# mclarsen/cuZFP

Measured on AMD Instinct MI355X. Metric: GB/s input encoded+decoded (device-resident), 3D f32 fixed-rate; % HBM peak, higher is better.
Workload: dtype f32; 1 GPU; 3d_float32_256^3_rate8; maxbits=512, parallelism=z-slab x1, stream_bytes_per_gpu=16777216

## Files before the change

### cuzfp_amd/csrc/zfp_block.hpp

```cpp
#pragma once

#include <math.h>
#include <stdint.h>

#if defined(__HIPCC__)
#include <hip/hip_runtime.h>
#define ZFP_HD __host__ __device__ __forceinline__
#else
#define ZFP_HD inline
#endif

#ifndef ZFP_STAMP
#define ZFP_STAMP(i)
#endif
#ifndef ZFP_COUNT_PLANE
#define ZFP_COUNT_PLANE(g0, fast, complete)
#endif
#ifndef ZFP_COUNT_PATH
#define ZFP_COUNT_PATH(id)
#endif

namespace cuzfp {


template <typename T> struct traits;
template <> struct traits<float> {
  typedef int32_t Int; typedef uint32_t UInt;
  static constexpr bool is_int = false;
  static constexpr int prec = 32, ebits = 8, ebias = 127;
};
template <> struct traits<double> {
  typedef int64_t Int; typedef uint64_t UInt;
  static constexpr bool is_int = false;
  static constexpr int prec = 64, ebits = 11, ebias = 1023;
};
template <> struct traits<int32_t> {
  typedef int32_t Int; typedef uint32_t UInt;
  static constexpr bool is_int = true;
  static constexpr int prec = 32, ebits = 0, ebias = 0;
};
template <> struct traits<int64_t> {
  typedef int64_t Int; typedef uint64_t UInt;
  static constexpr bool is_int = true;
  static constexpr int prec = 64, ebits = 0, ebias = 0;
};

template <typename UInt> struct nbmask;
template <> struct nbmask<uint32_t> { static constexpr uint32_t value = 0xaaaaaaaau; };
template <> struct nbmask<uint64_t> { static constexpr uint64_t value = 0xaaaaaaaaaaaaaaaaull; };

ZFP_HD uint64_t lowmask(unsigned n) { return n >= 64 ? ~0ull : ((1ull << n) - 1); }

struct WRaw {
  uint32_t a0, a1, a2;
};

ZFP_HD void sched_fence() {
#if defined(__HIP_DEVICE_COMPILE__)
  __builtin_amdgcn_sched_barrier(0);
#endif
}

ZFP_HD uint32_t launder(uint32_t x) {
#if defined(__HIP_DEVICE_COMPILE__)
  asm("" : "+v"(x));
#endif
  return x;
}
ZFP_HD uint32_t uniform_const(uint32_t x) {
#if defined(__HIP_DEVICE_COMPILE__)
  asm("" : "+s"(x));
#endif
  return x;
}
ZFP_HD uint64_t uniform_const64(uint64_t x) {
#if defined(__HIP_DEVICE_COMPILE__)
  asm("" : "+s"(x));
#endif
  return x;
}
ZFP_HD uint64_t launder(uint64_t x) {
#if defined(__HIP_DEVICE_COMPILE__)
  asm("" : "+v"(x));
#endif
  return x;
}

ZFP_HD unsigned ctz64(uint64_t x) { return (unsigned)__builtin_ctzll(x); }

ZFP_HD unsigned umin(unsigned a, unsigned b) { return a < b ? a : b; }


template <int DIMS> struct perm;
template <> struct perm<1> {
  ZFP_HD static constexpr int at(int i) { return i; }
};
template <> struct perm<2> {
  ZFP_HD static constexpr int at(int i) {
    return i == 0 ? 0 : i == 1 ? 1 : i == 2 ? 4 : i == 3 ? 5 : i == 4 ? 2 : i == 5 ? 8 :
           i == 6 ? 6 : i == 7 ? 9 : i == 8 ? 3 : i == 9 ? 12 : i == 10 ? 10 : i == 11 ? 7 :
           i == 12 ? 13 : i == 13 ? 11 : i == 14 ? 14 : 15;
  }
};
#define ZFP_I3(i, j, k) ((i) + 4 * ((j) + 4 * (k)))
template <> struct perm<3> {
  ZFP_HD static constexpr int at(int i) {
    constexpr int t[64] = {
      ZFP_I3(0,0,0),
      ZFP_I3(1,0,0), ZFP_I3(0,1,0), ZFP_I3(0,0,1),
      ZFP_I3(0,1,1), ZFP_I3(1,0,1), ZFP_I3(1,1,0),
      ZFP_I3(2,0,0), ZFP_I3(0,2,0), ZFP_I3(0,0,2),
      ZFP_I3(1,1,1),
      ZFP_I3(2,1,0), ZFP_I3(2,0,1), ZFP_I3(0,2,1), ZFP_I3(1,2,0), ZFP_I3(1,0,2), ZFP_I3(0,1,2),
      ZFP_I3(3,0,0), ZFP_I3(0,3,0), ZFP_I3(0,0,3),
      ZFP_I3(2,1,1), ZFP_I3(1,2,1), ZFP_I3(1,1,2),
      ZFP_I3(0,2,2), ZFP_I3(2,0,2), ZFP_I3(2,2,0),
      ZFP_I3(3,1,0), ZFP_I3(3,0,1), ZFP_I3(0,3,1), ZFP_I3(1,3,0), ZFP_I3(1,0,3), ZFP_I3(0,1,3),
      ZFP_I3(1,2,2), ZFP_I3(2,1,2), ZFP_I3(2,2,1),
      ZFP_I3(3,1,1), ZFP_I3(1,3,1), ZFP_I3(1,1,3),
      ZFP_I3(3,2,0), ZFP_I3(3,0,2), ZFP_I3(0,3,2), ZFP_I3(2,3,0), ZFP_I3(2,0,3), ZFP_I3(0,2,3),
      ZFP_I3(2,2,2),
      ZFP_I3(3,2,1), ZFP_I3(3,1,2), ZFP_I3(1,3,2), ZFP_I3(2,3,1), ZFP_I3(2,1,3), ZFP_I3(1,2,3),
      ZFP_I3(0,3,3), ZFP_I3(3,0,3), ZFP_I3(3,3,0),
      ZFP_I3(3,2,2), ZFP_I3(2,3,2), ZFP_I3(2,2,3),
      ZFP_I3(1,3,3), ZFP_I3(3,1,3), ZFP_I3(3,3,1),
      ZFP_I3(2,3,3), ZFP_I3(3,2,3), ZFP_I3(3,3,2),
      ZFP_I3(3,3,3)};
    return t[i];
  }
};
#undef ZFP_I3

template <int... I> struct seq {};
template <int N, int... I> struct seq_gen : seq_gen<N - 1, N - 1, I...> {};
template <int... I> struct seq_gen<0, I...> { typedef seq<I...> type; };
template <int N> using make_seq = typename seq_gen<N>::type;
template <int DIMS, int I> struct pidx { static constexpr int value = perm<DIMS>::at(I); };

template <int DIMS, typename UInt, int... I>
ZFP_HD void permute_fwd_add(const UInt* q, UInt* u, UInt nb, seq<I...>) {
  ((u[I] = q[pidx<DIMS, I>::value] + nb), ...);
}
ZFP_HD uint32_t from_negabinary(uint32_t u, uint32_t nb) {
#if defined(__HIP_DEVICE_COMPILE__)
  uint32_t r;
  asm("v_xad_u32 %0, %1, %2, %3" : "=v"(r) : "v"(u), "s"(nb), "v"(0u - nb));
  return r;
#else
  return (u ^ nb) - nb;
#endif
}
ZFP_HD uint64_t from_negabinary(uint64_t u, uint64_t nb) { return (u ^ nb) - nb; }

template <int DIMS, typename UInt, int... I>
ZFP_HD void permute_inv(const UInt* u, UInt* q, UInt nb, seq<I...>) {
  ((q[pidx<DIMS, I>::value] = from_negabinary(u[I], nb)), ...);
}
template <int DIMS, typename UInt, int... I>
ZFP_HD void permute_inv_copy(const UInt* u, UInt* q, seq<I...>) {
  ((q[pidx<DIMS, I>::value] = u[I]), ...);
}
template <int DIMS, typename UInt, int... I>
ZFP_HD void permute_inv_sub(const UInt* u, UInt* q, UInt nb, seq<I...>) {
  ((q[pidx<DIMS, I>::value] = u[I] - nb), ...);
}

template <int DIMS>
ZFP_HD unsigned precision(int emax, int prec) {
  int p = emax + 1074 + 2 * (DIMS + 1);
  p = p < 0 ? 0 : p;
  return (unsigned)(p < prec ? p : prec);
}


ZFP_HD uint32_t asr1(uint32_t v) { return (uint32_t)((int32_t)v >> 1); }
ZFP_HD uint64_t asr1(uint64_t v) { return (uint64_t)((int64_t)v >> 1); }

template <typename UInt>
ZFP_HD void fwd_lift(UInt& x, UInt& y, UInt& z, UInt& w) {
  x += w; x = asr1(x); w -= x;
  z += y; z = asr1(z); y -= z;
  x += z; x = asr1(x); z -= x;
  w += y; w = asr1(w); y -= w;
  w += asr1(y); y -= asr1(w);
}

template <typename UInt>
ZFP_HD void inv_lift(UInt& x, UInt& y, UInt& z, UInt& w) {
  UInt t;
  y += asr1(w); w -= asr1(y);
  t = w - y; y += w; w = t;
  t = x - z; z += x; x = t;
  t = z - y; y += z; z = t;
  t = x - w; w += x; x = t;
}

template <int DIMS, typename UInt>
ZFP_HD void fwd_xform(UInt* p) {
  if constexpr (DIMS == 1) {
    fwd_lift(p[0], p[1], p[2], p[3]);
  } else if constexpr (DIMS == 2) {
#pragma unroll
    for (int y = 0; y < 4; y++) fwd_lift(p[4 * y], p[4 * y + 1], p[4 * y + 2], p[4 * y + 3]);
#pragma unroll
    for (int x = 0; x < 4; x++) fwd_lift(p[x], p[x + 4], p[x + 8], p[x + 12]);
  } else {
#pragma unroll
    for (int zy = 0; zy < 16; zy++) fwd_lift(p[4 * zy], p[4 * zy + 1], p[4 * zy + 2], p[4 * zy + 3]);
#pragma unroll
    for (int z = 0; z < 4; z++)
#pragma unroll
      for (int x = 0; x < 4; x++) {
        UInt* q = p + 16 * z + x;
        fwd_lift(q[0], q[4], q[8], q[12]);
      }
#pragma unroll
    for (int yx = 0; yx < 16; yx++) fwd_lift(p[yx], p[yx + 16], p[yx + 32], p[yx + 48]);
  }
}

template <int DIMS, typename UInt>
ZFP_HD void inv_xform(UInt* p) {
  if constexpr (DIMS == 1) {
    inv_lift(p[0], p[1], p[2], p[3]);
  } else if constexpr (DIMS == 2) {
#pragma unroll
    for (int x = 0; x < 4; x++) inv_lift(p[x], p[x + 4], p[x + 8], p[x + 12]);
#pragma unroll
    for (int y = 0; y < 4; y++) inv_lift(p[4 * y], p[4 * y + 1], p[4 * y + 2], p[4 * y + 3]);
  } else {
#pragma unroll
    for (int yx = 0; yx < 16; yx++) inv_lift(p[yx], p[yx + 16], p[yx + 32], p[yx + 48]);
#pragma unroll
    for (int z = 0; z < 4; z++)
#pragma unroll
      for (int x = 0; x < 4; x++) {
        UInt* q = p + 16 * z + x;
        inv_lift(q[0], q[4], q[8], q[12]);
      }
#pragma unroll
    for (int zy = 0; zy < 16; zy++) inv_lift(p[4 * zy], p[4 * zy + 1], p[4 * zy + 2], p[4 * zy + 3]);
  }
}


ZFP_HD uint32_t bfi_v(uint32_t m, uint32_t a, uint32_t b) {
#if defined(__HIP_DEVICE_COMPILE__)
  uint32_t r;
  asm("v_bfi_b32 %0, %1, %2, %3" : "=v"(r) : "v"(m), "v"(a), "v"(b));
  return r;
#else
  return (a & m) | (b & ~m);
#endif
}

ZFP_HD uint32_t bfi(uint32_t m, uint32_t a, uint32_t b) {
#if defined(__HIP_DEVICE_COMPILE__)
  uint32_t r;
  asm("v_bfi_b32 %0, %1, %2, %3" : "=v"(r) : "s"(m), "v"(a), "v"(b));
  return r;
#else
  return (a & m) | (b & ~m);
#endif
}

ZFP_HD uint32_t nbfi(uint32_t m, uint32_t a, uint32_t b) {
#if defined(__HIP_DEVICE_COMPILE__)
  uint32_t r;
  asm("v_bitop3_b32 %0, %1, %2, %3 bitop3:0x35" : "=v"(r) : "s"(m), "v"(a), "v"(b));
  return r;
#else
  return ~((a & m) | (b & ~m));
#endif
}

ZFP_HD uint32_t bfi_notb(uint32_t m, uint32_t a, uint32_t b) {
#if defined(__HIP_DEVICE_COMPILE__)
  uint32_t r;
  asm("v_bitop3_b32 %0, %1, %2, %3 bitop3:0xc5" : "=v"(r) : "s"(m), "v"(a), "v"(b));
  return r;
#else
  return (a & m) | (~b & ~m);
#endif
}

ZFP_HD uint32_t perm_bytes(uint32_t b, uint32_t a, uint32_t sel) {
#if defined(__HIP_DEVICE_COMPILE__)
  return __builtin_amdgcn_perm(b, a, sel);
#else
  const uint64_t v = (uint64_t)a | ((uint64_t)b << 32);
  uint32_t r = 0;
  for (int i = 0; i < 4; i++) r |= (uint32_t)((v >> (8 * ((sel >> (8 * i)) & 7))) & 0xff) << (8 * i);
  return r;
#endif
}

enum { kInvNone = 0, kOddWords = 1, kOddBits = 2 };

template <int J>
ZFP_HD uint32_t opaque_shift() {
#if defined(__HIP_DEVICE_COMPILE__)
  uint32_t s;
  asm("s_mov_b32 %0, %1" : "=s"(s) : "i"(J));
  return s;
#else
  return J;
#endif
}
template <int J>
ZFP_HD void shl2(uint32_t& x, uint32_t& y, uint32_t sj) {
  const uint64_t r = ((uint64_t)x | ((uint64_t)y << 32)) << sj;
  x = (uint32_t)r;
  y = (uint32_t)(r >> 32);
}
template <int J>
ZFP_HD void shr2(uint32_t& x, uint32_t& y, uint32_t sj) {
  const uint64_t r = ((uint64_t)x | ((uint64_t)y << 32)) >> sj;
  x = (uint32_t)r;
  y = (uint32_t)(r >> 32);
}

template <int J, int INV = kInvNone>
ZFP_HD void transpose_stage(uint32_t* a, int rows, int r0 = 0) {
  constexpr uint32_t m = J == 16 ? 0x0000ffffu : J == 8 ? 0x00ff00ffu : J == 4 ? 0x0f0f0f0fu
                       : J == 2 ? 0x33333333u : 0x55555555u;
  if constexpr (J <= 4) {
    constexpr int D = J == 1 ? 2 : 1;
    const uint32_t sj = opaque_shift<J>();
#pragma unroll
    for (int i = 0; i < 32; i++) {
      if (i < r0 || i >= rows || (i & J) || (i & D)) continue;
      const int i2 = i + D;
      uint32_t h1 = a[i + J], h2 = a[i2 + J], l1 = a[i], l2 = a[i2];
      const uint32_t H1 = h1, H2 = h2;
      shl2<J>(h1, h2, sj);
      shr2<J>(l1, l2, sj);
      if constexpr (INV == kOddBits) {
        a[i] = bfi_notb(m, a[i], h1);
        a[i2] = bfi_notb(m, a[i2], h2);
        a[i + J] = bfi_notb(m, l1, H1);
        a[i2 + J] = bfi_notb(m, l2, H2);
      } else {
        a[i] = bfi(m, a[i], h1);
        a[i2] = bfi(m, a[i2], h2);
        a[i + J] = INV == kOddWords ? nbfi(m, l1, H1) : bfi(m, l1, H1);
        a[i2 + J] = INV == kOddWords ? nbfi(m, l2, H2) : bfi(m, l2, H2);
      }
    }
    return;
  }
#pragma unroll
  for (int i = 0; i < 32; i++) {
    if (i < r0 || i >= rows || (i & J)) continue;
    const uint32_t lo = a[i], hi = a[i + J];
    if constexpr (J == 16) {
      a[i] = perm_bytes(hi, lo, 0x05040100u);
      a[i + J] = perm_bytes(hi, lo, 0x07060302u);
    } else if constexpr (J == 8) {
      a[i] = perm_bytes(hi, lo, 0x06020400u);
      a[i + J] = perm_bytes(hi, lo, 0x07030501u);
    } else {
      if constexpr (INV == kOddBits) {
        a[i] = bfi_notb(m, lo, hi << J);
        a[i + J] = bfi_notb(m, lo >> J, hi);
      } else {
        a[i] = bfi(m, lo, hi << J);
        a[i + J] = INV == kOddWords ? nbfi(m, lo >> J, hi) : bfi(m, lo >> J, hi);
      }
    }
  }
}

template <int R, int INV = kInvNone>
ZFP_HD void transpose_tiles(uint32_t* a) {
  if constexpr (R >= 32) transpose_stage<16>(a, R);
  if constexpr (R >= 16) transpose_stage<8>(a, R);
  if constexpr (R >= 8) transpose_stage<4>(a, R);
  if constexpr (R >= 4) transpose_stage<2>(a, R);
  if constexpr (R >= 2) transpose_stage<1, INV>(a, R);
}

template <int H, int G, int R, bool VEC> struct plane_words;
template <int H, int G, int R> struct plane_words<H, G, R, false> {
  uint32_t a[H][G][R];
  ZFP_HD uint32_t get(int h, int g, int r) const { return a[h][g][r]; }
  ZFP_HD void set(int h, int g, int r, uint32_t x) { a[h][g][r] = x; }
  ZFP_HD void zero() {
#pragma unroll
    for (int h = 0; h < H; h++)
#pragma unroll
      for (int g = 0; g < G; g++)
#pragma unroll
        for (int r = 0; r < R; r++) a[h][g][r] = 0u;
  }
};
template <int H, int G, int R> struct plane_words<H, G, R, true> {
  typedef uint32_t vec __attribute__((ext_vector_type(R)));
  vec v[H][G];
  ZFP_HD uint32_t get(int h, int g, int r) const { return v[h][g][r]; }
  ZFP_HD void set(int h, int g, int r, uint32_t x) { v[h][g][r] = x; }
  ZFP_HD void zero() {
#pragma unroll
    for (int h = 0; h < H; h++)
#pragma unroll
      for (int g = 0; g < G; g++) v[h][g] = (vec)0u;
  }
};

template <typename UInt, int DIMS> struct planes {
  static constexpr int N = 1 << (2 * DIMS);
  static constexpr int H = sizeof(UInt) / 4;
  static constexpr int R = N < 32 ? N : 32;
  static constexpr int G = N / R;
  plane_words<H, G, R, (H == 2)> w;

  template <bool NEG_ODD = false>
  ZFP_HD void load(const UInt* u) {
    uint32_t t[H][N];
#pragma unroll
    for (int i = 0; i < N; i++) {
      t[0][i] = (uint32_t)u[i];
      if (H == 2) t[H - 1][i] = (uint32_t)((uint64_t)u[i] >> 32);
    }
#pragma unroll
    for (int h = 0; h < H; h++)
#pragma unroll
      for (int g = 0; g < G; g++) transpose_tiles<R, NEG_ODD ? kOddWords : kInvNone>(&t[h][g * R]);
#pragma unroll
    for (int h = 0; h < H; h++)
#pragma unroll
      for (int g = 0; g < G; g++)
#pragma unroll
        for (int r = 0; r < R; r++) w.set(h, g, r, t[h][g * R + r]);
  }

  template <bool NEG_ODD = false>
  ZFP_HD void store(UInt* u) const {
    uint32_t t[H][N];
#pragma unroll
    for (int h = 0; h < H; h++)
#pragma unroll
      for (int g = 0; g < G; g++)
#pragma unroll
        for (int r = 0; r < R; r++) t[h][g * R + r] = w.get(h, g, r);
#pragma unroll
    for (int h = 0; h < H; h++)
#pragma unroll
      for (int g = 0; g < G; g++) transpose_tiles<R, NEG_ODD ? kOddBits : kInvNone>(&t[h][g * R]);
#pragma unroll
    for (int i = 0; i < N; i++) {
      uint64_t x = t[0][i];
      if (H == 2) x |= (uint64_t)t[H - 1][i] << 32;
      u[i] = (UInt)x;
    }
  }

  ZFP_HD void zero() { w.zero(); }

  template <bool NEG_ODD = false>
  ZFP_HD void load_split(const UInt* u) {
    static_assert(H == 2 && N == 64, "3D 64-bit blocks");
    uint32_t t[H][N];
#pragma unroll
    for (int i = 0; i < N; i++) {
      t[0][i] = (uint32_t)u[i];
      t[1][i] = (uint32_t)((uint64_t)u[i] >> 32);
    }
#pragma unroll
    for (int g = 0; g < G; g++) {
      transpose_tiles<R, NEG_ODD ? kOddWords : kInvNone>(&t[1][g * R]);
      transpose_stage<16>(&t[0][g * R], R);
    }
#pragma unroll
    for (int h = 0; h < H; h++)
#pragma unroll
      for (int g = 0; g < G; g++)
#pragma unroll
        for (int r = 0; r < R; r++) w.set(h, g, r, t[h][g * R + r]);
  }
  template <bool NEG_ODD = false, bool UPPER = true>
  ZFP_HD void lo_part() {
    constexpr int INV = NEG_ODD ? kOddWords : kInvNone;
    constexpr int r0 = UPPER ? 16 : 0, r1 = UPPER ? 32 : 16;
#pragma unroll
    for (int g = 0; g < G; g++) {
      uint32_t t[R];
#pragma unroll
      for (int r = r0; r < r1; r++) t[r] = w.get(0, g, r);
      transpose_stage<8>(t, r1, r0);
      transpose_stage<4>(t, r1, r0);
      transpose_stage<2>(t, r1, r0);
      transpose_stage<1, INV>(t, r1, r0);
#pragma unroll
      for (int r = r0; r < r1; r++) w.set(0, g, r, t[r]);
    }
  }

  template <bool NEG_ODD = false>
  ZFP_HD void load_hi(const UInt* u) {
    static_assert(DIMS == 2 && H == 1, "2D 32-bit blocks");
    uint32_t d[8];
#pragma unroll
    for (int k = 0; k < 8; k++) d[k] = perm_bytes(u[k + 8], u[k], 0x07030602u);
    transpose_tiles<8, NEG_ODD ? kOddWords : kInvNone>(d);
#pragma unroll
    for (int k = 0; k < 8; k++) {
      w.set(0, 0, k, d[k] << 16);
      w.set(0, 0, k + 8, d[k]);
    }
  }
  template <bool NEG_ODD = false>
  ZFP_HD void store_hi(UInt* q) const {
    static_assert(DIMS == 2 && H == 1, "2D 32-bit blocks");
    uint32_t d[8];
#pragma unroll
    for (int k = 0; k < 8; k++) d[k] = perm_bytes(w.get(0, 0, k + 8), w.get(0, 0, k), 0x07030602u);
    transpose_tiles<8, NEG_ODD ? kOddBits : kInvNone>(d);
#pragma unroll
    for (int k = 0; k < 8; k++) {
      if constexpr (NEG_ODD) {
        q[k] = (d[k] - 0xaaaau) << 16;
        q[k + 8] = (d[k] & 0xffff0000u) - 0xaaaa0000u;
      } else {
        q[k] = d[k] << 16;
        q[k + 8] = d[k] & 0xffff0000u;
      }
    }
  }

  template <int h> ZFP_HD uint64_t get(int c) const {
    if constexpr (N == 64) return (uint64_t)w.get(h, 0, c) | ((uint64_t)w.get(h, 1, c) << 32);
    else return (w.get(h, 0, c % R) >> (R * (c / R))) & (uint32_t)lowmask(R);
  }
  ZFP_HD uint64_t get(int k) const {
    return (k >> 5) ? get<H - 1>(k & 31) : get<0>(k & 31);
  }
  template <int h> ZFP_HD uint32_t word(int c) const { return w.get(h, 0, c % R); }

  template <int h> ZFP_HD void set(int c, uint64_t x) {
    if constexpr (N == 64) {
      w.set(h, 0, c, (uint32_t)x);
      w.set(h, 1, c, (uint32_t)(x >> 32));
    } else {
      w.set(h, 0, c % R, w.get(h, 0, c % R) | ((uint32_t)x << (R * (c / R))));
    }
  }
  ZFP_HD void set(int k, uint64_t x) {
    if (k >> 5) set<H - 1>(k & 31, x);
    else set<0>(k & 31, x);
  }
};


template <int DIMS> struct plane_word { typedef uint32_t type; };
template <> struct plane_word<3> { typedef uint64_t type; };

ZFP_HD unsigned ctz(uint32_t x) { return (unsigned)__builtin_ctz(x); }
ZFP_HD unsigned ctz(uint64_t x) { return (unsigned)__builtin_ctzll(x); }

ZFP_HD unsigned ctz64_or_64(uint64_t x) {
#if defined(__HIP_DEVICE_COMPILE__)
  unsigned lo, hi;
  asm("v_ffbl_b32 %0, %1" : "=v"(lo) : "v"((uint32_t)x));
  asm("v_ffbl_b32 %0, %1" : "=v"(hi) : "v"((uint32_t)(x >> 32)));
  hi |= 32u;
  return lo < hi ? lo : hi;
#else
  const uint32_t lo = (uint32_t)x, hi = (uint32_t)(x >> 32);
  const unsigned zl = lo ? (unsigned)__builtin_ctz(lo) : 64u;
  const unsigned zh = hi ? 32u + (unsigned)__builtin_ctz(hi) : 64u;
  return zl < zh ? zl : zh;
#endif
}

ZFP_HD int uniform(int c) {
#if defined(__HIP_DEVICE_COMPILE__)
  return __builtin_amdgcn_readfirstlane(c);
#else
  return c;
#endif
}

ZFP_HD bool any_lane(bool p) {
#if defined(__HIP_DEVICE_COMPILE__) && !defined(CUZFP_LANE_EXIT)
  return __builtin_amdgcn_ballot_w64(p) != 0;
#else
  return p;
#endif
}

#ifndef CUZFP_PRIO_T2
#define CUZFP_PRIO_T2 17
#define CUZFP_PRIO_T1 9
#define CUZFP_PRIO_T0 1
#endif
#ifndef CUZFP_DPRIO_T2
#define CUZFP_DPRIO_T2 21
#define CUZFP_DPRIO_T1 11
#define CUZFP_DPRIO_T0 (-1)
#define CUZFP_DPRIO_AFTER 2
#endif
template <typename T, typename = void> struct prio_of {
  static constexpr bool value = true;
};
template <typename T> struct prio_of<T, decltype((void)T::kPrio)> {
  static constexpr bool value = T::kPrio;
};

template <typename T, typename = void> struct zero_inline_of {
  static constexpr bool value = false;
};
template <typename T> struct zero_inline_of<T, decltype((void)T::kZeroInline)> {
  static constexpr bool value = T::kZeroInline;
};

template <typename T, typename = void> struct put32_of {
  static constexpr bool value = false;
};
template <typename T> struct put32_of<T, decltype((void)T::kPut32)> {
  static constexpr bool value = T::kPut32;
};
template <typename W>
ZFP_HD auto wr_head(W& wr, uint64_t v, unsigned n) -> decltype(wr.head(v, n)) {
  wr.head(v, n);
}
template <typename W, typename... Ignored>
ZFP_HD void wr_head(W& wr, uint64_t v, unsigned n, Ignored...) {
  wr.put(v, n);
}

template <int T2, int T1, int T0>
ZFP_HD void progress_priority(int c) {
#if defined(__HIP_DEVICE_COMPILE__) && !defined(CUZFP_NO_PRIO)
  constexpr uint32_t kAt = (1u << T2) | (1u << T1) | (T0 >= 0 ? 1u << (T0 & 31) : 0u);
  if (__builtin_expect((kAt >> (c & 31)) & 1u, 0)) {
    if (c == T2) __builtin_amdgcn_s_setprio(2);
    else if (c == T1) __builtin_amdgcn_s_setprio(1);
    else __builtin_amdgcn_s_setprio(0);
  }
#else
  (void)c;
#endif
}

constexpr uint32_t spread_entry(uint32_t b) {
  uint32_t e = 0, p = 0;
  for (int i = 0; i < 8; i++) {
    if ((b >> i) & 1u) {
      e |= 3u << p;
      p += 2;
    } else {
      p += 1;
    }
  }
  return e;
}
struct SpreadLut {
  uint32_t e[256];
};
constexpr SpreadLut make_spread_lut() {
  SpreadLut t{};
  for (uint32_t b = 0; b < 256; b++) t.e[b] = spread_entry(b);
  return t;
}

struct SpreadTab {
  uint32_t e[512];
};
constexpr SpreadTab make_spread_tab() {
  SpreadTab t{};
  for (uint32_t b = 0; b < 256; b++) {
    uint32_t pop = 0;
    for (int i = 0; i < 8; i++) pop += (b >> i) & 1u;
    t.e[b] = (((spread_entry(b) << 1) | 1u) << 5) | (pop + 8u);
    t.e[256 + b] = spread_entry(b) << 1;
  }
  return t;
}

// ... 559 lines not shown
  const uint32_t d = parsed - b1;
  const bool done = ended | ((d == 0u) & (st != 0u));
  const bool cut = !done & ((int32_t)d >= 0);
  const uint32_t P = npos - (cut ? d : 0u);
  slow = (cut & (P > q)) | (!cut & (!done | ((int32_t)d > 1) | (npos > q)));
  uint64_t ones64 = ones | ((uint64_t)(cut ? 1u : 0u) << (P & 63u));
  uint32_t np = P + (cut ? 1u : 0u), take = umin(parsed, b1);
  if (__builtin_expect(any_lane(npos > q), 0)) {
    if (npos > q) {
      uint64_t o64 = ones;
      uint32_t o = implied_end(e1, e2, q, o64);
      if (ent_pos(e1) + ent_pos(e2) <= q) o = io;
      if (o <= b1) {
        slow = false;
        ones64 = o64;
        np = q + 1u;
        take = o;
      } else if (!cut) {
        slow = true;
      }
    }
  }
  ZFP_COUNT_PATH(slow ? (npos > q ? (cut ? 11 : 12) : (cut ? 13 : (!ended ? 14 : 15))) : 10);
  const PW hi = (PW)(~0ull << m);
  const PW x = (hi & ((PW)ones64 << nf)) | (~hi & (PW)w);
  n = nf + np;
  const unsigned adv = m + take;
  rd.pos += adv;
  bits -= adv;
  return x;
}

template <int DIMS, typename PW, typename Reader>
ZFP_HD PW decode_plane_lut(unsigned& bits, unsigned& n, Reader& rd, bool& slow) {
  constexpr unsigned N = 1u << (2 * DIMS);
  const unsigned nf = n < N - 1 ? n : N - 1;
  const unsigned m = umin(nf, bits);
  uint64_t w;
  uint32_t g;
  rd.windows(m, w, g);
  uint32_t e1, e2;
  if constexpr (DIMS == 1) {
    e1 = rd.chunk1_fast(g);
    e2 = 0;
  } else {
    uint32_t sel, e2a, e2b;
    rd.chunks_fast(g, e1, sel, e2a, e2b);
    e2 = perm_sel(e2b, e2a, sel);
  }
  return lut_finish<DIMS, PW>(bits, n, rd, slow, nf, m, w, e1, e2);
}

template <int DIMS, typename PW, typename Reader>
ZFP_HD PW decode_plane_any(unsigned& n, Reader& rd) {
  constexpr unsigned N = 1u << (2 * DIMS);
  const auto pos0 = rd.pos;
  const unsigned n0 = n;
  unsigned bits = rd.end - pos0;
  bool slow;
  PW x = decode_plane_lut<DIMS, PW>(bits, n, rd, slow);
  ZFP_COUNT_PATH(slow ? 6 : 5);
  if (__builtin_expect(any_lane(slow), 0)) {
    if (slow) {
      rd.init(pos0);
      n = n0;
      bits = rd.end - pos0;
      x = decode_plane<DIMS, PW>(bits, n, rd);
    }
  }
  n = umin(n, N - 1);
  return x;
}



template <int DIMS, typename PW, typename Reader>
ZFP_HD PW decode_plane_fast_any(unsigned& n, Reader& rd) {
  constexpr unsigned N = 1u << (2 * DIMS);
  const unsigned nf = n;
  WRaw wr;
  const uint32_t g = rd.window_g(nf, wr);
  uint32_t e1, e2, sel = 0, e2a = 0, e2b = 0;
  if constexpr (DIMS == 1)
    e1 = rd.chunk1_fast(g);
  else
    rd.chunks_fast(g, e1, sel, e2a, e2b);
  sched_fence();
  rd.lds_wait();
  sched_fence();
  const uint64_t w = rd.window_w_make(wr);
  if constexpr (DIMS == 1) {
    e2 = 0;
  } else {
    e2 = perm_sel(e2b, e2a, sel);
  }
  const uint32_t S = e1 + e2;
  const uint32_t nfp = nf + ent_pos(S);
  const int32_t rare = (int32_t)(S | ((N == 64 ? nfp : launder(nfp + (64u - N))) << 25));
  if (__builtin_expect(any_lane(rare < 0), 0)) {
    const auto pos0 = rd.pos;
    ZFP_COUNT_PATH((S & kMarkerBit) ? 16 : (nfp >= N) ? 17 : 18);
    unsigned bits = rd.end - rd.pos;
    bool slow;
    PW x = lut_finish<DIMS, PW>(bits, n, rd, slow, nf, umin(nf, bits), w, e1, e2);
    n = umin(n, N - 1);
    ZFP_COUNT_PATH(slow ? 2 : 1);
    if (any_lane(slow)) {
      if (slow) {
        rd.init(pos0);
        n = nf;
        bits = rd.end - pos0;
        x = decode_plane<DIMS, PW>(bits, n, rd);
        n = umin(n, N - 1);
      }
    }
    rd.lds_wait();
    return x;
  }
  ZFP_COUNT_PATH(0);
  const uint32_t ones = ent_ones(e1) | (ent_ones(e2) << ((e1 >> kPosShift) & 31u));
  PW x;
  if constexpr (sizeof(PW) == 8) {
    x = (PW)(w ^ (((w >> nf) ^ (uint64_t)ones) << nf));
  } else {
    x = merge_at<PW>(nf, ones, w);
  }
  n = nfp;
  rd.pos = umin(rd.pos + nf + ent_used(S), rd.end);
  return x;
}

template <int H, typename UInt, int DIMS, typename Reader>
ZFP_HD int decode_half(planes<UInt, DIMS>& P, unsigned& n, Reader& rd) {
  typedef typename plane_word<DIMS>::type PW;
  int c = 31;
  for (; c >= 1; c -= 2) {
    if (!any_lane(rd.pos < rd.end)) return c;
    if constexpr (prio_of<Reader>::value)
      progress_priority<CUZFP_DPRIO_T2, CUZFP_DPRIO_T1, CUZFP_DPRIO_T0>(uniform(c));
    PW xa, xb;
    xa = decode_plane_fast_any<DIMS, PW>(n, rd);
    xb = decode_plane_fast_any<DIMS, PW>(n, rd);
    ZFP_STAMP(4);
    const int u = uniform(c);
    P.template set<H>(u, xa);
    P.template set<H>(u - 1, xb);
  }
  return c;
}

#ifndef CUZFP_F64_SPLIT
#define CUZFP_F64_SPLIT 1
#endif
#ifndef CUZFP_EAGER_ZERO
constexpr bool kLazyZero = true;
#else
constexpr bool kLazyZero = false;
#endif
template <int H, int C, typename UInt, int DIMS>
ZFP_HD void zero_fixed(planes<UInt, DIMS>& P) {
  if constexpr (C >= 0) {
    P.template set<H>(C, 0);
    zero_fixed<H, C - 1>(P);
  }
}

template <int H, int C, bool PRI = true, typename UInt, int DIMS, typename Reader>
ZFP_HD int decode_half_fixed(planes<UInt, DIMS>& P, unsigned& n, Reader& rd) {
  typedef typename plane_word<DIMS>::type PW;
  if constexpr (C >= 1) {
    if (!any_lane(rd.pos < rd.end)) {
      if constexpr (kLazyZero && DIMS == 3) zero_fixed<H, C>(P);
      return C;
    }
#if defined(__HIP_DEVICE_COMPILE__) && !defined(CUZFP_NO_PRIO)
    if constexpr (prio_of<Reader>::value && PRI) {
      if constexpr (C == CUZFP_DPRIO_T2) __builtin_amdgcn_s_setprio(2);
      else if constexpr (C == CUZFP_DPRIO_T1) __builtin_amdgcn_s_setprio(1);
      else if constexpr (C == CUZFP_DPRIO_T0) __builtin_amdgcn_s_setprio(0);
    }
#endif
    const PW xa = decode_plane_fast_any<DIMS, PW>(n, rd);
    const PW xb = decode_plane_fast_any<DIMS, PW>(n, rd);
    ZFP_STAMP(4);
    P.template set<H>(C, xa);
    P.template set<H>(C - 1, xb);
    return decode_half_fixed<H, C - 2, PRI>(P, n, rd);
  }
  return C;
}


template <int H, typename UInt, int DIMS>
ZFP_HD void zero_planes(planes<UInt, DIMS>& P, int c) {
  if constexpr (kLazyZero && DIMS == 3)
    for (; c >= 0; c--) P.template set<H>(uniform(c), 0);
}

template <typename T, typename = void> struct has_dec1d {
  static constexpr bool value = false;
};
template <typename T> struct has_dec1d<T, decltype((void)&T::dec1d)> {
  static constexpr bool value = true;
};

template <int H, int C, typename UInt, typename Reader>
ZFP_HD void decode_planes_1d(planes<UInt, 1>& P, uint32_t& n12, Reader& rd) {
  if constexpr (C >= 0) {
    if constexpr (C & 1)
      if (!any_lane(rd.pos < rd.end)) return;
    const uint32_t c = umin(rd.end - rd.pos, 7u);
    const uint32_t e = rd.dec1d((rd.bits8() << 1) | ((c << 9) | n12));
    P.template set<H>(C, e & 15u);
    rd.pos += (e >> 4) & 15u;
    n12 = e & 0x3000u;
    decode_planes_1d<H, C - 1>(P, n12, rd);
  }
}

template <typename UInt, int DIMS, typename Reader>
ZFP_HD int decode_planes(planes<UInt, DIMS>& P, unsigned budget, Reader& rd) {
  constexpr int PREC = (int)sizeof(UInt) * 8;
  unsigned n = 0;
  rd.end = rd.pos + budget;
  if constexpr (!(kLazyZero && DIMS == 3)) P.zero();
  if constexpr (PREC == 32) {
    if constexpr (DIMS == 1 && has_dec1d<Reader>::value) {
      uint32_t n12 = 0;
      decode_planes_1d<0, 31>(P, n12, rd);
      return 31;
    }
    return decode_half_fixed<0, 31>(P, n, rd);
  } else {
    if constexpr (DIMS == 1 && has_dec1d<Reader>::value) {
      uint32_t n12 = 0;
      decode_planes_1d<1, 31>(P, n12, rd);
      decode_planes_1d<0, 31>(P, n12, rd);
      return 31;
    }
    zero_planes<1>(P, decode_half<1>(P, n, rd));
    zero_planes<0>(P, decode_half<0>(P, n, rd));
  }
  return 31;
}

template <typename UInt, int N>
ZFP_HD void cut_planes(UInt* v, unsigned maxprec) {
  constexpr unsigned PREC = (unsigned)sizeof(UInt) * 8;
  if (__builtin_expect(any_lane(maxprec != PREC), 0)) {
    const UInt m = (UInt)lowmask(PREC - maxprec);
    constexpr UInt NB = nbmask<UInt>::value;
#pragma unroll
    for (int i = 0; i < N; i++) v[i] = (v[i] & ~m) | (NB & m);
  }
}


template <typename Scalar> struct fp;

template <> struct fp<float> {
  template <int N>
  ZFP_HD static int emax(const float* f) {
    float m = 0.0f;
#pragma unroll
    for (int i = 0; i < N; i++) m = fmaxf(m, fabsf(f[i]));
    uint32_t b = __float_as_uint_(m);
    int E = (int)(b >> 23);
    if (b == 0) return -127;
    return E == 255 ? 0 : E - 126;
  }
  ZFP_HD static float pow2(int e) {
    if (e > 127) return __uint_as_float_(0x7f800000u);
    if (e >= -126) return __uint_as_float_((uint32_t)(e + 127) << 23);
    if (e >= -149) return __uint_as_float_(1u << (e + 149));
    return 0.0f;
  }
  ZFP_HD static int32_t to_int(float y) {
    return fabsf(y) < 2147483648.0f ? (int32_t)y : (int32_t)0x80000000u;
  }
  ZFP_HD static float from_int(int32_t q) { return (float)q; }
  ZFP_HD static uint32_t __float_as_uint_(float f) { union { float f; uint32_t u; } c; c.f = f; return c.u; }
  ZFP_HD static float __uint_as_float_(uint32_t u) { union { float f; uint32_t u; } c; c.u = u; return c.f; }
};

template <> struct fp<double> {
  template <int N>
  ZFP_HD static int emax(const double* f) {
    double m = 0.0;
#pragma unroll
    for (int i = 0; i < N; i++) m = fmax(m, fabs(f[i]));
    uint64_t b = as_u64(m);
    int E = (int)(b >> 52);
    if (b == 0) return -1023;
    return E == 2047 ? 0 : E - 1022;
  }
  ZFP_HD static double pow2(int e) {
    if (e > 1023) return as_f64(0x7ff0000000000000ull);
    if (e >= -1022) return as_f64((uint64_t)(e + 1023) << 52);
    if (e >= -1074) return as_f64(1ull << (e + 1074));
    return 0.0;
  }
  ZFP_HD static int64_t to_int(double y) {
    return fabs(y) < 9223372036854775808.0 ? (int64_t)y : (int64_t)0x8000000000000000ull;
  }
  ZFP_HD static double from_int(int64_t q) { return (double)q; }
  ZFP_HD static uint64_t as_u64(double f) { union { double f; uint64_t u; } c; c.f = f; return c.u; }
  ZFP_HD static double as_f64(uint64_t u) { union { double f; uint64_t u; } c; c.u = u; return c.f; }
};


#if defined(__HIP_DEVICE_COMPILE__)
template <int N>
__device__ __forceinline__ float absmax_nan(const float* f) {
  constexpr int C = N >= 16 ? 4 : 1;
  float m[C];
#pragma unroll
  for (int c = 0; c < C; c++) m[c] = 0.0f;
#pragma unroll
  for (int i = 0; i < N; i += 2) {
    float& a = m[(i / 2) % C];
    asm("v_maximum3_f32 %0, |%1|, |%2|, %0" : "+v"(a) : "v"(f[i]), "v"(f[i + 1]));
  }
  if constexpr (C == 4) {
    asm("v_maximum3_f32 %0, %0, %1, %2" : "+v"(m[0]) : "v"(m[1]), "v"(m[2]));
    asm("v_maximum3_f32 %0, %0, %1, %1" : "+v"(m[0]) : "v"(m[3]));
  }
  return m[0];
}
#endif

#if defined(__HIP_DEVICE_COMPILE__)
template <int N>
__device__ __forceinline__ void quantize_f32(const float* f, float s, bool fast, uint32_t* q) {
  typedef float f2 __attribute__((ext_vector_type(2)));
  if constexpr (N <= 16) fast = !any_lane(!fast);
  if (fast) {
    const f2 ss = {s, s};
#pragma unroll
    for (int i = 0; i < N; i += 2) {
      const f2 y = f2{f[i], f[i + 1]} * ss;
      q[i] = (uint32_t)(int32_t)y.x;
      q[i + 1] = (uint32_t)(int32_t)y.y;
    }
  }
  if (fast) {
  } else {
    const float lim = 2147483648.0f;
    const uint32_t imin = 0x80000000u;
#pragma unroll
    for (int i = 0; i < N; i += 2) {
      float a = f[i], b = f[i + 1];
      uint64_t m;
      uint32_t t;
      asm("v_mul_f32 %0, %0, %4\n\t"
          "v_mul_f32 %1, %1, %4\n\t"
          "v_cmp_gt_f32_e64 vcc, %5, |%0|\n\t"
          "v_cmp_gt_f32_e64 %2, %5, |%1|\n\t"
          "v_cvt_i32_f32 %3, %0\n\t"
          "v_cndmask_b32 %0, %6, %3, vcc\n\t"
          "v_cvt_i32_f32 %3, %1\n\t"
          "v_cndmask_b32_e64 %1, %6, %3, %2"
          : "+v"(a), "+v"(b), "=&s"(m), "=&v"(t)
          : "v"(s), "v"(lim), "v"(imin)
          : "vcc");
      q[i] = __builtin_bit_cast(uint32_t, a);
      q[i + 1] = __builtin_bit_cast(uint32_t, b);
    }
  }
}
#endif

template <typename Scalar, int DIMS, typename Writer>
ZFP_HD void encode_block(const Scalar* f, unsigned maxbits, Writer& wr) {
  typedef traits<Scalar> T;
  typedef typename T::Int Int;
  typedef typename T::UInt UInt;
  constexpr int N = 1 << (2 * DIMS);
  UInt q[N];
  unsigned maxprec = T::prec;
  (void)maxbits;
  if constexpr (!T::is_int) {
#if defined(__HIP_DEVICE_COMPILE__)
    bool finite = false;
    int emax;
    if constexpr (sizeof(Scalar) == 4 && N % 2 == 0) {
      const float mx = absmax_nan<N>((const float*)f);
      finite = __builtin_isfinite(mx);
      if (__builtin_expect(finite, 1)) {
        const uint32_t bm = __builtin_bit_cast(uint32_t, mx);
        emax = bm ? (int)(bm >> 23) - 126 : -127;
      } else {
        emax = fp<Scalar>::template emax<N>((const Scalar*)f);
      }
    } else {
      emax = fp<Scalar>::template emax<N>((const Scalar*)f);
    }
#else
    const int emax = fp<Scalar>::template emax<N>((const Scalar*)f);
#endif
    ZFP_STAMP(1);
    maxprec = precision<DIMS>(emax, T::prec);
    const unsigned e = maxprec ? (unsigned)(emax + T::ebias) : 0u;
    bool zero = !e;
    if (zero) maxprec = T::prec;
    if constexpr (zero_inline_of<Writer>::value) {
      if (!any_lane(!zero)) {
        wr.finish();
        return;
      }
      wr.mark_full(zero);
    } else if (zero) {
      wr.finish();
      return;
    }
    wr_head(wr, 2ull * e + 1, T::ebits + 1);
    Scalar s = (Scalar)fp<Scalar>::pow2(T::prec - 2 - emax);
    if constexpr (zero_inline_of<Writer>::value) s = zero ? (Scalar)0 : s;
#if defined(__HIP_DEVICE_COMPILE__)
    if constexpr (sizeof(Scalar) == 4 && N % 2 == 0) {
      quantize_f32<N>((const float*)f, (float)s, finite && (emax >= -97 || zero), (uint32_t*)q);
    } else
#endif
    {
#pragma unroll
      for (int i = 0; i < N; i++) q[i] = (UInt)fp<Scalar>::to_int(s * (Scalar)f[i]);
    }
  } else {
#pragma unroll
    for (int i = 0; i < N; i++) q[i] = (UInt)(Int)f[i];
  }
  fwd_xform<DIMS>(q);
  UInt u[N];
  constexpr UInt NB = nbmask<UInt>::value;
  permute_fwd_add<DIMS>(q, u, NB, make_seq<N>());
  if constexpr (sizeof(UInt) == 8 && !T::is_int) cut_planes<UInt, N>(u, maxprec);
  ZFP_STAMP(2);
#if defined(CUZFP_PROBE) && (CUZFP_PROBE == 1 || CUZFP_PROBE == 2)
  uint64_t acc = 0;
#if CUZFP_PROBE == 1
  planes<UInt, DIMS> P;
  P.load(u);
#pragma unroll
  for (int k = 0; k < (int)sizeof(UInt) * 8; k++) acc ^= (uint64_t)P.get(k) << (k & 7);
#else
#pragma unroll
  for (int i = 0; i < N; i++) acc ^= (uint64_t)u[i] << (i & 31);
#endif
  wr.put(acc, 64);
  (void)maxprec;
#else
  planes<UInt, DIMS> P;
  if constexpr (DIMS == 2 && sizeof(UInt) == 4) {
    P.template load_hi<true>(u);
    ZFP_STAMP(3);
    (void)maxprec;
    unsigned n = 0;
    if (encode_half_fixed<0, 31, true, 16>(P, n, wr)) {
      P.template load<true>(u);
      encode_half_fixed<0, 15>(P, n, wr);
    }
  } else if constexpr (CUZFP_F64_SPLIT && DIMS == 3 && sizeof(UInt) == 8 && zero_inline_of<Writer>::value) {
    planes<UInt, DIMS> PS;
    PS.template load_split<true>(u);
    ZFP_STAMP(3);
    unsigned n = 0;
    if (encode_half_fixed<1, 31>(PS, n, wr)) {
      PS.template lo_part<true, true>();
      if (encode_half_fixed<0, 31, false, 16>(PS, n, wr)) {
        PS.template lo_part<true, false>();
        encode_half_fixed<0, 15, false>(PS, n, wr);
      }
    }
  } else {
    P.template load<true>(u);
    ZFP_STAMP(3);
    encode_planes<UInt, DIMS>(P, wr);
  }
  ZFP_STAMP(4);
#endif
  wr.finish();
}

template <typename Scalar, int DIMS, typename Reader>
ZFP_HD bool decode_block(Scalar* f, unsigned maxbits, Reader& rd) {
  typedef traits<Scalar> T;
  typedef typename T::Int Int;
  typedef typename T::UInt UInt;
  constexpr int N = 1 << (2 * DIMS);
  unsigned budget = maxbits, maxprec = T::prec;
  int emax = 0;
  if constexpr (!T::is_int) {
    const uint64_t head = rd.peek();
    const bool coded = head & 1;
    if (!any_lane(coded)) return false;
    emax = (int)((head >> 1) & lowmask(T::ebits)) - T::ebias;
    const auto start = rd.pos;
    rd.skip(T::ebits + 1);
    maxprec = coded ? precision<DIMS>(emax, T::prec) : (unsigned)T::prec;
    budget = coded ? maxbits - (T::ebits + 1) : 0u;
    if (!coded) rd.pos = start + maxbits;
  }
  UInt u[N];
#if defined(CUZFP_PROBE) && CUZFP_PROBE == 2
  {
    const uint64_t base = rd.peek();
    (void)budget;
#pragma unroll
    for (int i = 0; i < N; i++) u[i] = (UInt)(base >> (i & 31)) + (UInt)i;
  }
#elif defined(CUZFP_PROBE) && CUZFP_PROBE == 1
  planes<UInt, DIMS> P;
  {
    const uint64_t base = rd.peek();
    (void)budget;
#pragma unroll
    for (int k = 0; k < (int)sizeof(UInt) * 8; k++)
      P.set(k, (typename plane_word<DIMS>::type)((base >> (k & 15)) ^ (uint64_t)k));
  }
  P.store(u);
#else
  planes<UInt, DIMS> P;
  const int unset = decode_planes<UInt, DIMS>(P, budget, rd);
  (void)unset;
#if defined(__HIP_DEVICE_COMPILE__) && !defined(CUZFP_NO_PRIO) && CUZFP_DPRIO_AFTER >= 0
  if constexpr (prio_of<Reader>::value) __builtin_amdgcn_s_setprio(CUZFP_DPRIO_AFTER);
#endif
  ZFP_STAMP(1);
  UInt q[N];
  constexpr UInt NB = nbmask<UInt>::value;
  if constexpr (DIMS == 2 && sizeof(UInt) == 4) {
    if (unset >= 15) {
      P.template store_hi<true>(u);
      permute_inv_copy<DIMS>(u, q, make_seq<N>());
    } else {
      P.template store<true>(u);
      permute_inv_sub<DIMS>(u, q, NB, make_seq<N>());
    }
    ZFP_STAMP(2);
  } else {
    P.template store<true>(u);
    if constexpr (sizeof(UInt) == 8 && !T::is_int) cut_planes<UInt, N>(u, maxprec);
    ZFP_STAMP(2);
    permute_inv_sub<DIMS>(u, q, NB, make_seq<N>());
  }
#endif
#if defined(CUZFP_PROBE) && (CUZFP_PROBE == 1 || CUZFP_PROBE == 2)
  UInt q[N];
  constexpr UInt NB = nbmask<UInt>::value;
  permute_inv<DIMS>(u, q, NB, make_seq<N>());
#endif
  inv_xform<DIMS>(q);
  ZFP_STAMP(3);
  if constexpr (!T::is_int) {
    const Scalar s = (Scalar)fp<Scalar>::pow2(emax - (T::prec - 2));
#if defined(__HIP_DEVICE_COMPILE__)
    if constexpr (sizeof(Scalar) == 4 && N % 2 == 0) {
      typedef float f2 __attribute__((ext_vector_type(2)));
      const f2 ss = {(float)s, (float)s};
#pragma unroll
      for (int i = 0; i < N; i += 2) {
        const f2 v = f2{(float)(Int)q[i], (float)(Int)q[i + 1]} * ss;
        f[i] = (Scalar)v.x;
        f[i + 1] = (Scalar)v.y;
      }
    } else
#endif
    if constexpr (sizeof(Scalar) == 8) {
#pragma unroll
      for (int i = 0; i < N; i++) {
        const int64_t v = (int64_t)(Int)q[i];
        const double d = __builtin_fma((double)(int32_t)(v >> 32), 4294967296.0, (double)(uint32_t)v);
        f[i] = (Scalar)(s * d);
      }
    } else {
#pragma unroll
      for (int i = 0; i < N; i++) f[i] = (Scalar)(s * (Scalar)(Int)q[i]);
    }
  } else {
#pragma unroll
    for (int i = 0; i < N; i++) f[i] = (Scalar)(Int)q[i];
  }
  return true;
}


ZFP_HD int pad_src(int i, int n) { return i < n ? i : (i == 3 ? 0 : n - 1); }


template <int DIMS>
ZFP_HD unsigned precision_variable(int emax, unsigned maxprec, int minexp) {
  int p = emax - minexp + 2 * (DIMS + 1);
  p = p < 0 ? 0 : p;
  return (unsigned)p < maxprec ? (unsigned)p : maxprec;
}

template <int DIMS>
ZFP_HD unsigned plane_bits(uint64_t x, unsigned& n) {
  constexpr unsigned N = 1u << (2 * DIMS);
  const uint64_t r = n < N ? x >> n : 0ull;
  const unsigned bl = r ? 64u - (unsigned)__builtin_clzll(r) : 0u;
  const unsigned nn = n + bl;
  const unsigned imp = (bl != 0u && nn == N) ? 1u : 0u;
  const unsigned len = n + (unsigned)__builtin_popcountll(r) + bl - imp + (nn < N ? 1u : 0u);
  n = nn;
  return len;
}

template <typename Scalar, int DIMS>
ZFP_HD unsigned block_length(const Scalar* f, unsigned maxprec, int minexp) {
  typedef traits<Scalar> T;
  typedef typename T::UInt UInt;
  constexpr int N = 1 << (2 * DIMS);
  static_assert(!T::is_int, "the variable-rate modes are defined for floats");
  const int emax = fp<Scalar>::template emax<N>(f);
  const unsigned p = precision_variable<DIMS>(emax, maxprec, minexp);
  if (!p || emax + T::ebias == 0) return 1u;
  const Scalar s = (Scalar)fp<Scalar>::pow2(T::prec - 2 - emax);
  UInt q[N], u[N];
#pragma unroll
  for (int i = 0; i < N; i++) q[i] = (UInt)fp<Scalar>::to_int(s * f[i]);
  fwd_xform<DIMS>(q);
  permute_fwd_add<DIMS>(q, u, nbmask<UInt>::value, make_seq<N>());
  planes<UInt, DIMS> P;
  P.template load<true>(u);
  unsigned len = 1u + T::ebits, n = 0;
#pragma unroll
  for (int k = T::prec - 1; k >= 0; k--) {
    unsigned nn = n;
    const unsigned l = plane_bits<DIMS>((uint64_t)P.get(k), nn);
    const bool coded = (unsigned)k + p >= (unsigned)T::prec;
    len += coded ? l : 0u;
    n = coded ? nn : n;
  }
  return len;
}

template <typename Scalar, int DIMS>
ZFP_HD constexpr unsigned max_block_bits(unsigned maxprec) {
  return 1u + traits<Scalar>::ebits + ((1u << (2 * DIMS)) - 1u) + (maxprec << (2 * DIMS));
}

}
```

Measured before the change: 1439 GB/s.

## Add 16-bit fast path for upper bit-plane tile transpose in 3D f32

For 3D 32-bit blocks, the plane store/load is split into two 32-coefficient tiles. When all lanes have zero upper rows in the second tile, the decoder uses a cheaper half-width transpose that reconstructs the second half as 16-bit values with the negabinary pattern in the upper bits. Otherwise it falls back to the full tile transpose. An encoder variant using packed 16-bit adds is also added but disabled by default. The intent is to cut transpose work in decode for low-rate blocks whose upper coefficients have few significant planes, at the cost of a wave-uniform check and extra branching.

Result: no change. 1446 GB/s, median of 6 (+0.5%).

```diff
diff --git a/cuzfp_amd/csrc/zfp_block.hpp b/cuzfp_amd/csrc/zfp_block.hpp
--- a/cuzfp_amd/csrc/zfp_block.hpp
+++ b/cuzfp_amd/csrc/zfp_block.hpp
@@ -141,6 +141,10 @@
 ZFP_HD void permute_fwd_add(const UInt* q, UInt* u, UInt nb, seq<I...>) {
   ((u[I] = q[pidx<DIMS, I>::value] + nb), ...);
 }
+template <int DIMS, typename UInt, int... I>
+ZFP_HD void permute_fwd_add_hi16(const UInt* q, UInt* u, UInt nb, seq<I...>) {
+  ((u[I] = q[pidx<DIMS, I>::value] + (I < 32 ? nb : (nb & 0xffffu))), ...);
+}
 ZFP_HD uint32_t from_negabinary(uint32_t u, uint32_t nb) {
 #if defined(__HIP_DEVICE_COMPILE__)
   uint32_t r;
@@ -292,6 +296,16 @@
   uint32_t r = 0;
   for (int i = 0; i < 4; i++) r |= (uint32_t)((v >> (8 * ((sel >> (8 * i)) & 7))) & 0xff) << (8 * i);
   return r;
+#endif
+}
+
+ZFP_HD uint32_t pk_add_u16(uint32_t a, uint32_t b) {
+#if defined(__HIP_DEVICE_COMPILE__)
+  uint32_t r;
+  asm("v_pk_add_u16 %0, %1, %2" : "=v"(r) : "v"(a), "s"(b));
+  return r;
+#else
+  return ((a + (b & 0xffffu)) & 0xffffu) | ((a & 0xffff0000u) + (b & 0xffff0000u));
 #endif
 }
 
@@ -525,6 +539,81 @@
         q[k] = d[k] << 16;
         q[k + 8] = d[k] & 0xffff0000u;
       }
+    }
+  }
+
+  ZFP_HD static bool fits_hi16(const UInt* v) {
+    static_assert(DIMS == 3 && H == 1, "3D 32-bit blocks");
+    uint32_t m = 0;
+#pragma unroll
+    for (int i = 0; i < R; i++) m = m > v[R + i] ? m : v[R + i];
+    return m < 0x10000u;
+  }
+  template <int g, bool NEG_ODD = false>
+  ZFP_HD void load_tile(const UInt* u) {
+    static_assert(H == 1, "32-bit blocks");
+    uint32_t t[R];
+#pragma unroll
+    for (int i = 0; i < R; i++) t[i] = u[g * R + i];
+    transpose_tiles<R, NEG_ODD ? kOddWords : kInvNone>(t);
+#pragma unroll
+    for (int r = 0; r < R; r++) w.set(0, g, r, t[r]);
+  }
+  template <int g, bool NEG_ODD = false>
+  ZFP_HD void store_tile(UInt* u) const {
+    static_assert(H == 1, "32-bit blocks");
+    uint32_t t[R];
+#pragma unroll
+    for (int r = 0; r < R; r++) t[r] = w.get(0, g, r);
+    transpose_tiles<R, NEG_ODD ? kOddBits : kInvNone>(t);
+#pragma unroll
+    for (int i = 0; i < R; i++) u[g * R + i] = t[i];
+  }
+  ZFP_HD uint32_t load_hi16_head(const UInt* v) {
+    static_assert(DIMS == 3 && H == 1, "3D 32-bit blocks");
+    uint32_t t[R];
+#pragma unroll
+    for (int i = 0; i < R; i++) t[i] = v[R + i];
+    transpose_stage<16>(t, R);
+#pragma unroll
+    for (int r = 0; r < R; r++) w.set(0, 1, r, t[r]);
+    return hi16_rows();
+  }
+  template <bool UPPER>
+  ZFP_HD void load_hi16_part() {
+    constexpr int r0 = UPPER ? 16 : 0, r1 = UPPER ? 32 : 16;
+    uint32_t t[R];
+#pragma unroll
+    for (int r = r0; r < r1; r++) t[r] = UPPER ? pk_add_u16(w.get(0, 1, r), 0xaaaaaaaau) : w.get(0, 1, r);
+    transpose_stage<8>(t, r1, r0);
+    transpose_stage<4>(t, r1, r0);
+    transpose_stage<2>(t, r1, r0);
+    transpose_stage<1, kOddWords>(t, r1, r0);
+#pragma unroll
+    for (int r = r0; r < r1; r++) w.set(0, 1, r, t[r]);
+  }
+  ZFP_HD void load_hi16_lo() { load_hi16_part<false>(); }
+  ZFP_HD void load_hi16_hi() { load_hi16_part<true>(); }
+  ZFP_HD uint32_t hi16_rows() const {
+    static_assert(DIMS == 3 && H == 1, "3D 32-bit blocks");
+    uint32_t o = 0;
+#pragma unroll
+    for (int r = 16; r < R; r++) o |= w.get(0, 1, r);
+    return o;
+  }
+  ZFP_HD void store_hi16(UInt* u) const {
+    static_assert(DIMS == 3 && H == 1, "3D 32-bit blocks");
+    uint32_t t[16];
+#pragma unroll
+    for (int r = 0; r < 16; r++) t[r] = w.get(0, 1, r);
+    transpose_stage<8>(t, 16);
+    transpose_stage<4>(t, 16);
+    transpose_stage<2>(t, 16);
+    transpose_stage<1, kOddBits>(t, 16);
+#pragma unroll
+    for (int i = 0; i < 16; i++) {
+      u[R + i] = (t[i] & 0xffffu) | 0xaaaa0000u;
+      u[R + i + 16] = (t[i] >> 16) | 0xaaaa0000u;
     }
   }
 
@@ -1390,6 +1479,12 @@
 #ifndef CUZFP_F64_SPLIT
 #define CUZFP_F64_SPLIT 1
 #endif
+#ifndef CUZFP_HI16
+#define CUZFP_HI16 1
+#endif
+#ifndef CUZFP_HI16_ENC
+#define CUZFP_HI16_ENC 0
+#endif
 #ifndef CUZFP_EAGER_ZERO
 constexpr bool kLazyZero = true;
 #else
@@ -1670,7 +1765,13 @@
   fwd_xform<DIMS>(q);
   UInt u[N];
   constexpr UInt NB = nbmask<UInt>::value;
-  permute_fwd_add<DIMS>(q, u, NB, make_seq<N>());
+#if CUZFP_HI16 && CUZFP_HI16_ENC && !(defined(CUZFP_PROBE) && (CUZFP_PROBE == 1 || CUZFP_PROBE == 2))
+  constexpr bool kHi16 = DIMS == 3 && sizeof(UInt) == 4;
+#else
+  constexpr bool kHi16 = false;
+#endif
+  if constexpr (kHi16) permute_fwd_add_hi16<DIMS>(q, u, NB, make_seq<N>());
+  else permute_fwd_add<DIMS>(q, u, NB, make_seq<N>());
   if constexpr (sizeof(UInt) == 8 && !T::is_int) cut_planes<UInt, N>(u, maxprec);
   ZFP_STAMP(2);
 #if defined(CUZFP_PROBE) && (CUZFP_PROBE == 1 || CUZFP_PROBE == 2)
@@ -1709,6 +1810,13 @@
         encode_half_fixed<0, 15, false>(PS, n, wr);
       }
     }
+  } else if constexpr (kHi16) {
+    P.template load_tile<0, true>(u);
+    const uint32_t hi = P.load_hi16_head(u);
+    P.load_hi16_lo();
+    if (any_lane(hi != 0)) P.load_hi16_hi();
+    ZFP_STAMP(3);
+    encode_planes<UInt, DIMS>(P, wr);
   } else {
     P.template load<true>(u);
     ZFP_STAMP(3);
@@ -1775,6 +1883,12 @@
       permute_inv_sub<DIMS>(u, q, NB, make_seq<N>());
     }
     ZFP_STAMP(2);
+  } else if constexpr (CUZFP_HI16 && DIMS == 3 && sizeof(UInt) == 4) {
+    P.template store_tile<0, true>(u);
+    if (!any_lane(P.hi16_rows() != 0)) P.store_hi16(u);
+    else P.template store_tile<1, true>(u);
+    ZFP_STAMP(2);
+    permute_inv_sub<DIMS>(u, q, NB, make_seq<N>());
   } else {
     P.template store<true>(u);
     if constexpr (sizeof(UInt) == 8 && !T::is_int) cut_planes<UInt, N>(u, maxprec);
```
